# luo-ziyuan/NeRF_Signature

Hardware: AMD Instinct MI355X
Metric: training rays/sec @4096 rays (hotdog, 32-bit msg) (higher is better)
Workload: dtype f32 (hash gather, compositing) + fp16 MFMA with f32 accumulate (MLPs); 1 GPU; BASELINE configs[1]: Blender/hotdog-like S0, --wtmk_tcnn, 4096 content + 32x12x12 block rays, 32-bit msg; content_rays=4096, block_rays_total=4608, block_rays_this_rank=4608, message_dim=32, parallelism=dp1, capacity_overflow=False, recaptured_with_more_headroom_after_warmup=False, execution=hipgraph, graph_segments=1

## Files before the change

### include/nerfsig.h

```cpp
#ifndef NERFSIG_H_
#define NERFSIG_H_

#include <stddef.h>
#include <stdint.h>

#ifdef __cplusplus
extern "C" {
#endif

#define NSIG_OK 0
#define NSIG_ERR_ARG 1
#define NSIG_ERR_LAUNCH 2

#define NSIG_TABLE_ROWS (1u << 19)
#define NSIG_BASE_LEVELS 16
#define NSIG_MAX_MESSAGE_DIM 64

typedef void *nsig_stream_t;

int nsig_abi_version(void);
const char *nsig_last_error(void);


int rm_near_far_from_aabb(const float *rays_o, const float *rays_d, const float *aabb, uint32_t N, float min_near,
// ... 133 lines not shown
#define NSIG_PLANES_MIXED 1
int field_fwd(const float *xyzs, const float *dirs, uint32_t M, float bound, const float *const *base_tables_host,
              const float *S, const void *packed, float *sigmas, float *rgbs, float *geo_feat, uint32_t *masks,
              const void *planes, int planes_layout, nsig_stream_t stream);

size_t hg_planes_bytes(uint32_t M);
int hg_encode_planes(const float *xyzs, uint32_t M, float bound, const float *const *base_tables_host, const float *S,
                     void *planes, nsig_stream_t stream);
int hg_encode_planes_rows(const float *xyzs, uint32_t M_capacity, const uint32_t *rows_dev, float bound,
                          const float *const *base_tables_host, const float *S, void *planes, nsig_stream_t stream);
int hg_encode_planes_mixed(const float *xyzs, uint32_t M_capacity, const uint32_t *rows_dev, float bound, const float *const *base_tables_host,
                           const float *S, void *planes, nsig_stream_t stream);
int field_fwd_rows(const float *xyzs, const float *dirs, uint32_t M_capacity, const uint32_t *rows_dev, float bound,
                   const float *const *base_tables_host, const float *S, const void *packed, float *sigmas, float *rgbs, const void *planes,
                   int planes_layout, nsig_stream_t stream);

int hg_warm_tables(const float *const *base_tables_host, const float *S, float *sink, nsig_stream_t stream);

int hg_encode_codebook_plane(const float *xyzs, uint32_t M, float bound, const float *S, void *planes, int planes_layout, void *plan_to_reset,
                             nsig_stream_t stream);

int field_color_fwd(const float *dirs, const float *geo_feat, uint32_t M, const void *packed, float *rgbs,
                    nsig_stream_t stream);

int field_bwd(const float *xyzs, uint32_t M, float bound, const float *grad_sigmas, const float *grad_rgbs,
              const float *sigmas, const float *rgbs, const uint32_t *masks, const void *packed, float *G,
              float *dfeat_out, float *rec_out, nsig_stream_t stream);
int field_bwd_planned(const float *xyzs, uint32_t M, float bound, const float *grad_sigmas, const float *grad_rgbs,
                      const float *sigmas, const float *rgbs, const uint32_t *masks, const void *packed, void *plan,
                      nsig_stream_t stream);

int opt_adam_dense(uint32_t n, float *const *params_host, const float *const *grads_host, float *const *exp_avg_host,
                   float *const *exp_avg_sq_host, float *const *steps_host, const uint32_t *numel_host, const float *lr, float beta1,
                   float beta2, float eps, float grad_scale, float *scratch, nsig_stream_t stream);
int opt_adam_dense_host(uint32_t n, float *const *params_host, const float *const *grads_host, float *const *exp_avg_host,
// ... 122 lines not shown
```

### nerf_signature_amd/_native.py

```python
import ctypes
import os

import torch

_PKG = os.path.dirname(os.path.abspath(__file__))
LIB_PATH = os.path.join(_PKG, "lib", "libnerfsig.so")

_c = ctypes
_vp, _u32, _fl, _int, _sz = _c.c_void_p, _c.c_uint32, _c.c_float, _c.c_int, _c.c_size_t

SIGNATURES = {
    "nsig_abi_version": [],
    "nsig_last_error": [],
    "nsig_host_device_pointer": [_vp],
    "rg_sample_rays": [_vp, _u32, _vp, _fl, _fl, _fl, _fl, _u32, _u32, _u32, _vp, _u32, _u32, _c.c_uint64, _vp, _vp, _vp, _vp, _vp, _vp],
    "rg_get_rays": [_vp, _fl, _fl, _fl, _fl, _u32, _u32, _vp, _u32, _u32, _vp, _vp, _vp],
    "rm_near_far_from_aabb": [_vp, _vp, _vp, _u32, _fl, _vp, _vp, _vp],
    "rm_sph_from_ray": [_vp, _vp, _fl, _u32, _vp, _vp],
    "rm_morton3D": [_vp, _u32, _vp, _vp],
    "rm_morton3D_invert": [_vp, _u32, _vp, _vp],
    "rm_packbits": [_vp, _u32, _fl, _vp, _vp],
    "rg_refresh_draw_scratch_bytes": [_u32, _u32],
    "rg_refresh_begin": [_vp, _u32, _vp],
    "rg_refresh_draw": [_vp, _vp, _u32, _u32, _vp, _vp, _c.c_uint64, _vp, _u32, _vp],
# ... 9 lines not shown
    "rm_march_train_write": [_vp, _vp, _fl, _fl, _u32, _u32, _u32, _u32, _u32, _vp, _vp, _vp, _vp, _vp, _vp, _vp, _vp, _vp],
    "rm_march_train_count_nf": [_vp, _vp, _vp, _fl, _vp, _fl, _fl, _u32, _u32, _u32, _u32, _vp, _vp, _vp, _vp, _vp, _vp],
    "rm_march_train_scan_write_max_rays": [],
    "rm_march_train_scan_write": [_vp, _vp, _fl, _fl, _u32, _u32, _u32, _u32, _u32, _vp, _vp, _vp, _vp, _vp, _vp, _vp, _vp, _vp, _vp],
    "rm_composite_train_fwd": [_vp, _vp, _vp, _vp, _u32, _u32, _fl, _vp, _vp, _vp, _vp],
    "rm_composite_train_bwd": [_vp, _vp, _vp, _vp, _vp, _vp, _vp, _vp, _u32, _u32, _fl, _vp, _vp, _vp],
    "rm_march": [_u32, _u32, _vp, _vp, _vp, _vp, _fl, _fl, _u32, _u32, _u32, _vp, _vp, _vp, _vp, _vp, _vp, _vp, _u32, _vp],
    "rm_composite": [_u32, _u32, _fl, _vp, _vp, _vp, _vp, _vp, _vp, _vp, _vp, _vp],
    "rm_compact_alive": [_vp, _u32, _vp, _vp, _vp],
    "rm_eval_begin": [_u32, _vp, _vp, _vp],
    "rm_eval_march": [_vp, _u32, _vp, _vp, _vp, _vp, _fl, _fl, _u32, _u32, _u32, _vp, _vp, _vp, _vp, _vp, _vp, _vp],
    "rm_eval_composite": [_vp, _u32, _fl, _fl, _vp, _vp, _vp, _vp, _vp, _vp, _vp, _vp, _vp],
    "rm_eval_compact": [_vp, _u32, _u32, _vp, _vp, _vp],
    "hg_encode_planes_rows": [_vp, _u32, _vp, _fl, _vp, _vp, _vp, _vp],
    "hg_encode_planes_mixed": [_vp, _u32, _vp, _fl, _vp, _vp, _vp, _vp],
    "field_fwd_rows": [_vp, _vp, _u32, _vp, _fl, _vp, _vp, _vp, _vp, _vp, _vp, _int, _vp],
    "hg_codebook_presum": [_vp, _u32, _vp, _vp],
    "hg_codebook_presum_sel": [_vp, _vp, _u32, _vp, _vp],
    "hg_encode_fwd": [_vp, _u32, _vp, _vp, _vp, _vp],
    "hg_codebook_encode_fwd": [_vp, _u32, _vp, _u32, _vp, _vp],
    "hg_codebook_bwd": [_vp, _u32, _vp, _vp, _vp],
    "hg_scatter_sliced": [_vp, _u32, _vp, _vp],
    "hg_fanout_grad": [_vp, _vp, _u32, _int, _vp],
    "hg_level_lookup": [_vp, _u32, _fl, _vp, _vp, _vp],
    "opt_codebook_adam": [_vp, _vp, _vp, _vp, _u32, _fl, _fl, _fl, _vp, _vp, _fl, _vp],
    "opt_codebook_adam_sel": [_vp, _vp, _vp, _vp, _vp, _vp, _u32, _vp, _fl, _fl, _fl, _fl, _vp, _vp],
    "opt_codebook_adam_sel_next": [_vp, _vp, _vp, _vp, _vp, _vp, _u32, _vp, _fl, _fl, _fl, _fl, _vp, _vp, _vp, _vp],
    "mlp_packed_bytes": [],
    "mlp_get_precision": [],
    "mlp_set_precision": [_int],
    "mlp_get_pipelined": [],
    "mlp_set_pipelined": [_int],
    "mlp_pack_weights": [_vp, _vp, _vp, _vp],
    "hg_planes_bytes": [_u32],
    "hg_encode_planes": [_vp, _u32, _fl, _vp, _vp, _vp, _vp],
    "hg_warm_tables": [_vp, _vp, _vp, _vp],
    "hg_encode_codebook_plane": [_vp, _u32, _fl, _vp, _vp, _int, _vp, _vp],
    "field_fwd": [_vp, _vp, _u32, _fl, _vp, _vp, _vp, _vp, _vp, _vp, _vp, _vp, _int, _vp],
    "field_color_fwd": [_vp, _vp, _u32, _vp, _vp, _vp],
    "opt_adam_dense_host": [_u32, _vp, _vp, _vp, _vp, _vp, _vp, _vp, _fl, _fl, _fl, _fl, _vp],
    "opt_adam_dense": [_u32, _vp, _vp, _vp, _vp, _vp, _vp, _vp, _fl, _fl, _fl, _fl, _vp, _vp],
    "rm_composite_train_finish_fwd": [_vp, _vp, _vp, _vp, _u32, _u32, _fl, _vp, _vp, _vp, _u32, _vp, _vp, _vp, _vp, _vp, _vp],
    "rm_composite_train_finish_bwd": [_vp, _vp, _vp, _vp, _vp, _vp, _vp, _vp, _vp, _u32, _u32, _u32, _fl, _u32, _vp, _vp, _vp],
    "rm_finish_fwd": [_vp, _vp, _vp, _vp, _vp, _vp, _u32, _u32, _vp, _vp, _vp],
    "rm_finish_bwd": [_vp, _vp, _vp, _vp, _vp, _vp, _u32, _u32, _vp, _vp, _vp],
    "loop_step_begin": [_vp, _u32, _vp, _u32, _u32, _vp, _vp, _vp],
    "wm_loss_fwd": [_vp, _vp, _u32, _vp, _vp, _u32, _fl, _fl, _fl, _vp, _vp, _vp, _vp],
    "wm_loss_bwd": [_vp, _vp, _vp, _fl, _fl, _vp, _u32, _vp, _u32, _vp, _vp, _vp],
    "dec_bn_gelu_fwd": [_vp, _vp, _vp, _u32, _u32, _u32, _fl, _vp, _vp, _vp],
    "dec_bn_gelu_bwd": [_vp, _vp, _vp, _vp, _vp, _u32, _u32, _u32, _vp, _vp, _vp, _vp],
    "dec_workspace_bytes": [_u32, _u32, _u32, _u32],
    "dec_forward": [_vp, _u32, _vp, _vp, _vp, _u32, _u32, _u32, _u32, _fl, _vp, _vp, _vp, _vp],
# ... 134 lines not shown
```

### nerf_signature_amd/csrc/field.hip

```cpp
#include <cstdlib>
#include <cstring>
#include <mutex>
#include <unordered_set>
#include "fieldmlp.h"

#include <stdlib.h>

namespace nsig {


__device__ inline float fwd_weight(int frag, int lane, int j, const float *__restrict__ sp, const float *__restrict__ cp) {
    const int r = lane & 31, h = lane >> 5;
    if (frag < F1) {
        const int rb = (frag - F0) >> 1, ks = (frag - F0) & 1;
        return sp[kSigmaW1 + (32 * rb + r) * 32 + 16 * ks + 8 * h + j];
    }
    if (frag < F2) return r < 16 ? sp[kSigmaW2 + r * 64 + k_from_acc(frag - F1, h, j)] : 0.0f;
    if (frag < F3) {
        const int rb = (frag - F2) >> 1, ks = (frag - F2) & 1;
        int cin;
        if (ks == 0) cin = 8 * h + j;
        else { const int rho = row_of_reg(h, j); cin = rho == 0 ? 31 : 15 + rho; }
        return cp[kColorW1 + (32 * rb + r) * 32 + cin];
    }
// ... 136 lines not shown
        if (m >= lim) continue;
        const uint32_t ml = min(m, M - 1);
        const float3 pt = *reinterpret_cast<const float3 *>(xyzs + 3 * (size_t)ml);
        const float x = (pt.x + bound) / two_b, y = (pt.y + bound) / two_b, z = (pt.z + bound) / two_b;
        for (int i = 0; i < n_levels; ++i) {
            const int l = tab.level[slot][i];
            const bool half_out = mixed && l < kHalfLevels;
            float2 *out = !mixed ? planes + (size_t)l * stride + m
                                 : (half_out ? reinterpret_cast<float2 *>(reinterpret_cast<uint32_t *>(planes) + (size_t)l * stride + m) : mixed_f32_plane(planes, stride, l) + m);
            encode_tile_level(reinterpret_cast<const float2 *>(l == NSIG_BASE_LEVELS ? S : base.p[l]), geom.cell[l], xs, x, y, z, out, half_out, mixed);
        }
    }
}

__global__ void __launch_bounds__(256) k_encode_codebook_plane(const float *__restrict__ xyzs, uint32_t M, float bound, float cell, const float *__restrict__ S,
                                                               float2 *__restrict__ plane, uint32_t stride, BinHeader *__restrict__ reset) {
    if (reset != nullptr && blockIdx.x == 0 && threadIdx.x == 0) reset->gmax_bits = 0;
    const uint32_t m = blockIdx.x * 256 + threadIdx.x;
    if (m >= stride) return;
    const uint32_t ml = min(m, M - 1);
    const float two_b = 2.0f * bound;
    const float3 pt = *reinterpret_cast<const float3 *>(xyzs + 3 * (size_t)ml);
    const float x = (pt.x + bound) / two_b, y = (pt.y + bound) / two_b, z = (pt.z + bound) / two_b;
    encode_tile_level(reinterpret_cast<const float2 *>(S), cell, threadIdx.x & 1u, x, y, z, plane + m);
}

template <typename P, bool kMixed>
__device__ inline void field_fwd_pipelined(const char *lds, int lane, const float *__restrict__ dirs, uint32_t M, bool add_codebook,
                                           const float2 *__restrict__ planes, uint32_t stride, float *__restrict__ sigmas, float *__restrict__ rgbs,
                                           uint32_t *__restrict__ masks) {
    static_assert(!kMixed || P::kMfmaPerProduct == 1, "mixed plane sets carry fp16 operands: the fp16 MLP only");
    constexpr size_t kHalf = kFwdBytes;
    const int p = lane & 31, h = lane >> 5;
    const uint32_t n_tiles = ceil_div(M, 32u);
// ... 664 lines not shown
    NSIG_REQUIRE(sink != nullptr, "hg_warm_tables: sink is one writable float (never written)");
    TablePtrs base{};
    if (int e = fill_base_tables(base_tables_host, base, "hg_warm_tables")) return e;
    k_warm_tables<<<8 * 128, 256, 0, as_stream(stream)>>>(base, S, default_slots(S != nullptr), sink);
    return check_launch("hg_warm_tables");
}

NSIG_EXPORT size_t hg_planes_bytes(uint32_t M) { return (size_t)(NSIG_BASE_LEVELS + 1) * ceil_div(M, 32u) * 32u * sizeof(float2); }

static int check_layout(int layout, const char *who) {
    NSIG_REQUIRE(layout == NSIG_PLANES_F32 || layout == NSIG_PLANES_MIXED, "%s: planes_layout must be NSIG_PLANES_F32 (0) or NSIG_PLANES_MIXED (1)", who);
    return NSIG_OK;
}

static int encode_planes_impl(const float *xyzs, uint32_t M, float bound, const float *const *base_tables_host, const float *S, void *planes,
                              const uint32_t *rows_dev, nsig_stream_t stream, bool mixed = false) {
    if (M == 0) return NSIG_OK;
    NSIG_REQUIRE(xyzs && planes, "hg_encode_planes: null pointer");
    NSIG_REQUIRE(bound > 0.0f, "hg_encode_planes: bound must be positive");
    NSIG_REQUIRE((reinterpret_cast<uintptr_t>(planes) & 7) == 0, "hg_encode_planes: planes must be 8-byte aligned");
    TablePtrs base{};
    if (int e = fill_base_tables(base_tables_host, base, "hg_encode_planes")) return e;
    const uint32_t stride = ceil_div(M, 32u) * 32u;
    const SlotTable tab = default_slots(S != nullptr);
    int covered[NSIG_BASE_LEVELS + 1] = {};
    for (int s = 0; s < 8; ++s)
        for (int i = 0; i < tab.n[s]; ++i) covered[tab.level[s][i]] += 1;
    for (int l = 0; l < NSIG_BASE_LEVELS + (S != nullptr ? 1 : 0); ++l)
        NSIG_REQUIRE(covered[l] == 1, "hg_encode_planes: level %d is assigned to %d slots", l, covered[l]);
    NSIG_REQUIRE(S != nullptr || covered[NSIG_BASE_LEVELS] == 0, "hg_encode_planes: slot table names the codebook level but S is NULL");
    const uint32_t tiles = ceil_div(stride, 256u);
    const uint32_t per_slot = tiles < 8192u ? tiles : 8192u;
    if (mixed) k_encode_planes<true><<<per_slot * 8, 256, 0, as_stream(stream)>>>(xyzs, M, bound, base, make_level_geom(), S, reinterpret_cast<float2 *>(planes), stride, tab, rows_dev);
    else k_encode_planes<false><<<per_slot * 8, 256, 0, as_stream(stream)>>>(xyzs, M, bound, base, make_level_geom(), S, reinterpret_cast<float2 *>(planes), stride, tab, rows_dev);
    return check_launch("hg_encode_planes");
}

NSIG_EXPORT int hg_encode_planes_mixed(const float *xyzs, uint32_t M_capacity, const uint32_t *rows_dev, float bound, const float *const *base_tables_host,
                                       const float *S, void *planes, nsig_stream_t stream) {
    NSIG_REQUIRE(mlp_precision() == 1, "hg_encode_planes_mixed: the mixed layout carries the fp16 MLP's operands (mlp_set_precision(1))");
    return encode_planes_impl(xyzs, M_capacity, bound, base_tables_host, S, planes, rows_dev, stream, true);
}

NSIG_EXPORT int hg_encode_planes(const float *xyzs, uint32_t M, float bound, const float *const *base_tables_host, const float *S, void *planes,
                                 nsig_stream_t stream) {
    return encode_planes_impl(xyzs, M, bound, base_tables_host, S, planes, nullptr, stream);
}

NSIG_EXPORT int hg_encode_planes_rows(const float *xyzs, uint32_t M_capacity, const uint32_t *rows_dev, float bound, const float *const *base_tables_host,
                                      const float *S, void *planes, nsig_stream_t stream) {
    NSIG_REQUIRE(rows_dev != nullptr, "hg_encode_planes_rows: null row count");
    return encode_planes_impl(xyzs, M_capacity, bound, base_tables_host, S, planes, rows_dev, stream);
}

NSIG_EXPORT int hg_encode_codebook_plane(const float *xyzs, uint32_t M, float bound, const float *S, void *planes, int planes_layout, void *plan_to_reset,
                                         nsig_stream_t stream) {
    if (M == 0) return NSIG_OK;
    if (int e = check_layout(planes_layout, "hg_encode_codebook_plane")) return e;
    NSIG_REQUIRE(xyzs && S && planes, "hg_encode_codebook_plane: null pointer");
    NSIG_REQUIRE(bound > 0.0f, "hg_encode_codebook_plane: bound must be positive");
    NSIG_REQUIRE((reinterpret_cast<uintptr_t>(planes) & 7) == 0, "hg_encode_codebook_plane: planes must be 8-byte aligned");
    NSIG_REQUIRE(plan_to_reset == nullptr || (reinterpret_cast<uintptr_t>(plan_to_reset) & 15) == 0, "hg_encode_codebook_plane: plan must be 16-byte aligned");
    const uint32_t stride = ceil_div(M, 32u) * 32u;
    float2 *plane = planes_layout == NSIG_PLANES_MIXED ? mixed_f32_plane(planes, stride, NSIG_BASE_LEVELS) : reinterpret_cast<float2 *>(planes) + (size_t)NSIG_BASE_LEVELS * stride;
    k_encode_codebook_plane<<<ceil_div(stride, 256u), 256, 0, as_stream(stream)>>>(xyzs, M, bound, make_level_geom().cell[NSIG_BASE_LEVELS], S, plane, stride,
                                                                                  reinterpret_cast<BinHeader *>(plan_to_reset));
    return check_launch("hg_encode_codebook_plane");
}

static int field_fwd_impl(const float *xyzs, const float *dirs, uint32_t M, float bound, const float *const *base_tables_host,
                          const float *S, const void *packed, float *sigmas, float *rgbs, float *geo_feat, uint32_t *masks,
                          const void *planes, int planes_layout, const uint32_t *rows_dev, nsig_stream_t stream) {
    if (M == 0) return NSIG_OK;
    NSIG_REQUIRE(xyzs && packed && sigmas, "field_fwd: null pointer");
    NSIG_REQUIRE(rgbs == nullptr || dirs != nullptr, "field_fwd: dirs is required when rgbs is requested");
    NSIG_REQUIRE(bound > 0.0f, "field_fwd: bound must be positive");
    NSIG_REQUIRE((reinterpret_cast<uintptr_t>(packed) & 15) == 0, "field_fwd: packed must be 16-byte aligned");
    TablePtrs base{};
    if (int e = fill_base_tables(base_tables_host, base, "field_fwd")) return e;
    const char *pk = reinterpret_cast<const char *>(packed);
    hipStream_t st = as_stream(stream);
    const bool f16 = mlp_precision() == 1;
// ... 151 lines not shown
```

### nerf_signature_amd/fieldops.py

```python
import os

import torch
from torch.autograd import Function
from torch.amp import custom_bwd, custom_fwd

from . import _native as nv

T_ROWS = 1 << 19
MASK_WORDS = 6

_fwd32 = custom_fwd(device_type="cuda", cast_inputs=torch.float32)
_bwd = custom_bwd(device_type="cuda")


def message_bits(message):
    if message is None:
        return None
    if isinstance(message, torch.Tensor):
        return tuple(int(v) for v in message.detach().to("cpu", torch.float32).tolist())
    return tuple(int(v) for v in message)


def select_tables(tables, bits):
    if len(tables) != 2 * len(bits):
# ... 96 lines not shown
def field_forward(xyzs, dirs, bound, base_tables, S, packed, want_rgb=True, want_geo=False, want_masks=False, planes=None, fixed=None):
    xyzs = xyzs.contiguous().float()
    M, dev = xyzs.shape[0], xyzs.device
    sigmas = torch.empty(M, dtype=torch.float32, device=dev)
    rgbs = torch.empty(M, 3, dtype=torch.float32, device=dev) if want_rgb else None
    geo = torch.empty(M, 15, dtype=torch.float32, device=dev) if want_geo else None
    masks = torch.empty((M + 31) // 32 * 32, MASK_WORDS, dtype=torch.int32, device=dev) if want_masks else None
    if want_rgb:
        dirs = dirs.contiguous().float()
    use_planes = (M >= PLANES_MIN_POINTS) if planes is None else bool(planes)
    base_ptrs = nv.ptr_array([_check_table(t.detach(), "base table") for t in base_tables])
    ws, layout = None, PLANES_F32
    if fixed is not None:
        fixed.check(xyzs, bound, base_tables)
        ws, layout = fixed.planes, fixed.layout
        reset = nv.ptr(fixed.plan.buf) if want_masks else None
        if S is not None:
            nv.call("hg_encode_codebook_plane", nv.ptr(xyzs), M, float(bound), nv.ptr(S), nv.ptr(ws), layout, reset, nv.stream())
    elif use_planes:
        ws = torch.empty(int(nv.fn("hg_planes_bytes")(M)), dtype=torch.uint8, device=dev)
        layout = encode_planes(xyzs, M, bound, base_ptrs, S, ws)
    nv.call("field_fwd", nv.ptr(xyzs), nv.ptr(dirs) if want_rgb else None, M, float(bound), base_ptrs, nv.ptr(S), nv.ptr(packed),
            nv.ptr(sigmas), nv.ptr(rgbs), nv.ptr(geo), nv.ptr(masks), nv.ptr(ws), layout, nv.stream())
    return sigmas, rgbs, geo, masks


def field_color(dirs, geo_feat, packed):
    dirs = dirs.contiguous().float()
    geo_feat = geo_feat.contiguous().float()
    M = dirs.shape[0]
    rgbs = torch.empty(M, 3, dtype=torch.float32, device=dirs.device)
# ... 104 lines not shown
                torch.cuda.current_stream().wait_event(self.ready)
            self.ready = None


class _KeptPlan:

    def __init__(self, M, buf):
        self.M, self.buf, self.launched, self.ready = M, buf, True, None

    def join(self):
        pass


class FixedPoints:

    def __init__(self, xyzs, bound, base_tables):
        self.M, self.bound = int(xyzs.shape[0]), float(bound)
        self.xyzs_ptr = xyzs.data_ptr()
        self.planes = torch.empty(int(nv.fn("hg_planes_bytes")(self.M)), dtype=torch.uint8, device=xyzs.device)
        self.plan = _KeptPlan(self.M, torch.empty(int(nv.fn("hg_scatter_plan_bytes")(self.M)), dtype=torch.uint8, device=xyzs.device))
        self.refreshes = 0
        self.refresh(xyzs, base_tables)

    @staticmethod
    def _tables_key(base_tables):
        return tuple((t.data_ptr(), t._version) for t in base_tables) + (mixed_planes(),)

    def refresh(self, xyzs, base_tables):
        if xyzs.data_ptr() != self.xyzs_ptr or xyzs.shape[0] != self.M:
            raise ValueError("FixedPoints.refresh: these are not the points the cache was built for")
        base_ptrs = nv.ptr_array([_check_table(t.detach(), "base table") for t in base_tables])
        self.layout = encode_planes(xyzs, self.M, self.bound, base_ptrs, None, self.planes)
        nv.call("hg_scatter_plan", nv.ptr(xyzs), self.M, self.bound, nv.ptr(self.plan.buf), nv.stream())
        self.key = self._tables_key(base_tables)
        self.refreshes += 1

    def check(self, xyzs, bound, base_tables):
        if xyzs.data_ptr() != self.xyzs_ptr or xyzs.shape[0] != self.M or float(bound) != self.bound:
            raise ValueError("FixedPoints: the field pass was handed other points than the cache was built for")
        if self._tables_key(base_tables) != self.key and not torch.cuda.is_current_stream_capturing():
            self.refresh(xyzs, base_tables)


def field_backward_planned(xyzs, bound, g_sigma, g_rgb, sigmas, rgbs, masks, packed, plan, G):
    plan.join()
    nv.call("field_bwd_planned", nv.ptr(xyzs), plan.M, float(bound), nv.ptr(g_sigma.contiguous().float()), nv.ptr(g_rgb.contiguous().float()),
            nv.ptr(sigmas), nv.ptr(rgbs), nv.ptr(masks), nv.ptr(packed), nv.ptr(plan.buf), nv.stream())
    nv.call("hg_scatter_planned", nv.ptr(plan.buf), plan.M, nv.ptr(G), nv.stream())
# ... 74 lines not shown
    __slots__ = ("base", "sel")

    def __init__(self, base, sel):
        self.base, self.sel = list(base), list(sel)


class _FieldFunction(Function):

    @staticmethod
    @_fwd32
    def forward(ctx, xyzs, dirs, bound, packed, S, sink, tabs, fixed, *diff):
        base, sel = tabs.base, tabs.sel
        n_sel = len(sel)
        need_grad = n_sel > 0 and len(diff) > 0
        xyzs = xyzs.contiguous().float()
        if fixed is not None:
            ctx.plan = fixed.plan if need_grad else None
        else:
            ctx.plan = ScatterPlan(xyzs, bound) if need_grad and xyzs.shape[0] >= binned_min_points() else None
        sigmas, rgbs, _, masks = field_forward(xyzs, dirs, bound, base, S, packed, want_masks=need_grad, fixed=fixed)
        ctx.bound, ctx.n_diff, ctx.need_grad, ctx.sink = bound, len(diff), need_grad, sink
        if need_grad:
            ctx.mlp_precision = nv.fn("mlp_get_precision")()
            ctx.save_for_backward(xyzs, sigmas, rgbs, masks, packed)
            if sink is not None:
                sink.selected = list(sel)
                ctx.sink_selected = sink.selected
        return sigmas, rgbs

    @staticmethod
    @_bwd
# ... 137 lines not shown
```

### nerf_signature_amd/network.py

```python
import torch

from . import fieldops as fo
from . import tcnn_compat as tcnn
from .hash_encoding import HashEmbedder
from .hash_encoding_wtmk_bit import HashEmbedder as HashEmbedder_msg
from .hidden_models import get_hidden_decoder_multi_views, normalize_img
from .renderer import NeRFRenderer


def _data_parallel():
    import torch.distributed as dist
    return dist.is_available() and dist.is_initialized() and dist.get_world_size() > 1


class NeRFNetwork(NeRFRenderer):
    def __init__(self, num_layers=2, hidden_dim=64, geo_feat_dim=15, num_layers_color=3, hidden_dim_color=64, bound=1, message_dim=16,
                 n_views=1, finetune_decoder=False, **kwargs):
        super().__init__(bound, **kwargs)
        if (num_layers, hidden_dim, geo_feat_dim, num_layers_color, hidden_dim_color) != (2, 64, 15, 3, 64):
            raise NotImplementedError("the native field network implements the reference's default architecture: "
                                      "sigma 32->64->1+15, color 16+15->64->64->3")
        self.finetune_decoder = finetune_decoder
        self.num_layers, self.hidden_dim, self.geo_feat_dim = num_layers, hidden_dim, geo_feat_dim
        self.num_layers_color, self.hidden_dim_color = num_layers_color, hidden_dim_color
# ... 178 lines not shown
        if capacity is None:
            capacity = self._count_points(o, d, dt_gamma, max_steps)
        rec = self.march_ahead(rays_o, rays_d, dt_gamma, max_steps, capacity=capacity)
        if loop_capacity is None and int(rec["counter"][0]) > capacity:
            capacity = raymarching.padded_point_count(int(rec["counter"][0]))
            rec = self.march_ahead(rays_o, rays_d, dt_gamma, max_steps, capacity=capacity)
        if rec.get("fixed") is None:
            rec["fixed"] = fo.FixedPoints(rec["xyzs"], self.bound, self.encoder.tables())
        else:
            rec["fixed"].refresh(rec["xyzs"], self.encoder.tables())
        rec["fixed_args"] = (dt_gamma, max_steps)
        rec["rays_ref"] = (rays_o, rays_d)
        rec["grid_key"] = self.grid_key()
        return rec

    def density(self, x, message=None):
        selected, _, S = self._select(message)
        if torch.is_grad_enabled() and x.is_cuda and len(selected) and any(t.requires_grad for t in selected):
            sigma, geo = fo.density_apply(x, self.bound, self._packed(), self.encoder.tables(), selected, S, self.grad_sink, self.sigma_net.params)
            return {"sigma": sigma, "geo_feat": geo}
        sigma, _, geo, _ = fo.field_forward(x, None, self.bound, self.encoder.tables(), S, self._packed(), want_rgb=False, want_geo=True)
        return {"sigma": sigma, "geo_feat": geo}

    def color(self, x, d, mask=None, geo_feat=None, **kwargs):
        grad = torch.is_grad_enabled() and geo_feat is not None and geo_feat.requires_grad and d.is_cuda
        one = (lambda dd, gg: fo.color_apply(dd, gg, self._packed(), self.color_net.params)) if grad else (lambda dd, gg: fo.field_color(dd, gg, self._packed()))
        if mask is not None:
            rgbs = torch.zeros(mask.shape[0], 3, dtype=torch.float32, device=x.device)
            if not mask.any():
                return rgbs
# ... 13 lines not shown
```

### nerf_signature_amd/renderer.py

```python
import math
import os

import numpy as np
import torch
import torch.nn as nn

from . import _native as nv
from . import raymarching


def custom_meshgrid(*args):
    return torch.meshgrid(*args, indexing="ij")


def sample_pdf(bins, weights, n_samples, det=False):
    B, T = bins.shape
    mass = weights + 1e-5
    cdf = torch.zeros(B, T, dtype=mass.dtype, device=mass.device)
    torch.cumsum(mass / mass.sum(-1, keepdim=True), -1, out=cdf[:, 1:])
    if det:
        q = ((torch.arange(n_samples, dtype=mass.dtype) + 0.5) / n_samples).to(mass.device).expand(B, n_samples)
    else:
        q = torch.rand(B, n_samples).to(mass.device)
    q = q.contiguous()
# ... 229 lines not shown
        if differentiable:
            rgbs = rgb_all * (weights > 1e-4).unsqueeze(-1)
        else:
            rgbs = self.color(pts.reshape(-1, 3), dirs_of(pts), mask=(weights > 1e-4).reshape(-1), geo_feat=geo.reshape(N * T, -1)).view(N, T, 3)
        weights_sum = weights.sum(dim=-1)
        depth = torch.sum(weights * ((z - nears) / span).clamp(0, 1), dim=-1)
        image = torch.sum(weights.unsqueeze(-1) * rgbs, dim=-2) + (1 - weights_sum).unsqueeze(-1) * bg_color
        return {"depth": depth.view(*prefix), "image": image.view(*prefix, 3), "weights_sum": weights_sum}



    @staticmethod
    def _rays_key(o, d):
        return (o.data_ptr(), o._version, d.data_ptr(), d._version, o.shape[0])

    def march_ahead(self, rays_o, rays_d, dt_gamma=0, max_steps=1024, perturb=False, phase="all", capacity=None, noises=None):
        if not hasattr(self, "_marched"):
            self._marched = {}
        prefix, o, d = self._flatten_rays(rays_o, rays_d)
        if capacity is None:
            capacity = getattr(self, "point_capacity", None)
            capacity = capacity.get(o.shape[0]) if capacity else None
        if capacity is None or not o.is_cuda:
            raise RuntimeError("march_ahead needs point_capacity for this ray count (see trainer.GraphedWatermarkLoop.prepare) and CUDA rays")
        rec = next((r for r in self._marched.values() if r["ptrs"] == (o.data_ptr(), d.data_ptr(), o.shape[0]) and r["capacity"] == capacity), None)
        if rec is None:
            N, dev = o.shape[0], o.device
            f32 = dict(dtype=torch.float32, device=dev)
            rec = {"ptrs": (o.data_ptr(), d.data_ptr(), N), "capacity": capacity, "nears": torch.empty(N, **f32), "fars": torch.empty(N, **f32),
                   "xyzs": torch.empty(capacity, 3, **f32), "dirs": torch.empty(capacity, 3, **f32), "deltas": torch.empty(capacity, 2, **f32),
                   "rays": torch.empty(N, 3, dtype=torch.int32, device=dev), "counter": torch.zeros(2, dtype=torch.int32, device=dev), "key": None,
                   "counts": torch.empty(N, dtype=torch.int32, device=dev), "t_rec": torch.empty(N * int(max_steps), **f32), "max_steps": int(max_steps),
                   "noises": None}
        if rec["max_steps"] != int(max_steps):
            raise ValueError("march_ahead: max_steps changed for rays that were marched before")
        N = o.shape[0]
        geom = (float(self.bound), float(dt_gamma), int(max_steps), N, int(self.cascade), int(self.grid_size))
        if phase in ("all", "count") and not raymarching.fused_limits():
            raymarching.near_far_into(o, d, self.aabb_train, self.min_near, rec["nears"], rec["fars"])
            rec["noises"] = noises if noises is not None else (torch.rand(N, dtype=torch.float32, device=o.device) if perturb else None)
            nv.call("rm_march_train_count", nv.ptr(o), nv.ptr(d), nv.ptr(self.density_bitfield), *geom, nv.ptr(rec["nears"]), nv.ptr(rec["fars"]),
                    nv.ptr(rec["noises"]), nv.ptr(rec["counts"]), nv.ptr(rec["t_rec"]), nv.stream())
        elif phase in ("all", "count"):
            rec["noises"] = noises if noises is not None else (torch.rand(N, dtype=torch.float32, device=o.device) if perturb else None)
            nv.call("rm_march_train_count_nf", nv.ptr(o), nv.ptr(d), nv.ptr(self.aabb_train), float(self.min_near), nv.ptr(self.density_bitfield), *geom,
                    nv.ptr(rec["noises"]), nv.ptr(rec["nears"]), nv.ptr(rec["fars"]), nv.ptr(rec["counts"]), nv.ptr(rec["t_rec"]), nv.stream())
        if phase in ("all", "write"):
            if N <= raymarching.scan_write_max_rays():
                nv.call("rm_march_train_scan_write", nv.ptr(o), nv.ptr(d), geom[0], geom[1], geom[2], N, geom[4], geom[5], capacity, nv.ptr(rec["nears"]),
                        nv.ptr(rec["noises"]), nv.ptr(rec["t_rec"]), nv.ptr(rec["counts"]), nv.ptr(rec["rays"]), nv.ptr(rec["counter"]), nv.ptr(rec["xyzs"]),
                        nv.ptr(rec["dirs"]), nv.ptr(rec["deltas"]), nv.stream())
            else:
                nv.call("rm_march_train_scan", nv.ptr(rec["counts"]), N, nv.ptr(rec["rays"]), nv.ptr(rec["counter"]), nv.stream())
                nv.call("rm_march_train_write", nv.ptr(o), nv.ptr(d), geom[0], geom[1], geom[2], N, geom[4], geom[5], capacity, nv.ptr(rec["nears"]),
                        nv.ptr(rec["noises"]), nv.ptr(rec["t_rec"]), nv.ptr(rec["rays"]), nv.ptr(rec["counter"]), nv.ptr(rec["xyzs"]), nv.ptr(rec["dirs"]),
                        nv.ptr(rec["deltas"]), nv.stream())
        self._marched = {k: r for k, r in self._marched.items() if r is not rec}
        rec["key"] = self._rays_key(o, d)
        self._marched[rec["key"]] = rec
        return rec

    def drop_marched(self):
        self._marched = {}

    def premarch(self, rays_o, rays_d, dt_gamma=0, max_steps=1024):
        import weakref
        prefix, o, d = self._flatten_rays(rays_o, rays_d)
        nears, fars = raymarching.near_far_from_aabb(o, d, self.aabb_train, self.min_near)
        counter = self.step_counter[self.local_step % 16]
        self.local_step += 1
        counter.zero_()
# ... 40 lines not shown
            if bg is not None:
                weights_sum, depth, image = out
                return {"depth": depth.view(*prefix), "image": image.view(*prefix, 3), "weights_sum": weights_sum}
            weights_sum, depth, image = out
        else:
            weights_sum, depth, image = self._march_and_composite_eval(o, d, message, nears, fars, dt_gamma, perturb, max_steps, T_thresh)
        image, depth = self._finish(prefix, image, depth, weights_sum, bg_color, nears, fars)
        results = {"depth": depth, "image": image}
        if self.training:
            results["weights_sum"] = weights_sum
        return results

    def _march_and_composite_train(self, o, d, message, nears, fars, dt_gamma, perturb, force_all_rays, max_steps, T_thresh, finish=None,
                                   marched=None, limits=None):
        if marched is not None:
            fixed = marched.get("fixed")
            if fixed is not None:
                sigmas, rgbs = self(marched["xyzs"], marched["dirs"], message, fixed=fixed)
            else:
                sigmas, rgbs = self(marched["xyzs"], marched["dirs"], message)
            sigmas = sigmas if self.density_scale == 1 else self.density_scale * sigmas
            if finish is not None:
                return _CompositeFinish.apply(sigmas, rgbs, marched["deltas"], marched["rays"], nears, fars, finish, T_thresh)
            return raymarching.composite_rays_train(sigmas, rgbs, marched["deltas"], marched["rays"], T_thresh)
        counter = self.step_counter[self.local_step % 16]
        self.local_step += 1
        capacity = getattr(self, "point_capacity", None)
        capacity = capacity.get(o.shape[0]) if capacity else None
        if not (capacity is not None and force_all_rays):
            counter.zero_()
        if capacity is not None and force_all_rays:
            xyzs, dirs, deltas, rays = raymarching.march_rays_train_capacity(o, d, self.bound, self.density_bitfield, self.cascade,
                                                                            self.grid_size, nears, fars, counter, capacity, perturb,
# ... 253 lines not shown
```

### nerf_signature_amd/trainer.py

```python
import ctypes
import os

import numpy as np
import torch
import torch.nn.functional as F

from . import _native as nv
from . import fieldops as fo
from . import dp
from .capture import SegmentedCapture, warm_up
from .dp import GradExchange, exchange_active, world_size
from .distortion import DistortionLayer, host_uniform, scaled_width
from .hidden_models import normalize_img, set_grad_arena, set_weights_stream


def loss_w_bce(decoded, keys, temp=10.0):
    return F.binary_cross_entropy_with_logits(decoded * temp, keys, reduction="mean")


def loss_w_mse(decoded, keys, temp=10.0):
    return torch.mean((decoded * temp - (2 * keys - 1)) ** 2)


class _WatermarkLoss(torch.autograd.Function):
# ... 336 lines not shown
        p = preds.detach().cpu().numpy() if torch.is_tensor(preds) else preds
        t = truths.detach().cpu().numpy() if torch.is_tensor(truths) else truths
        self.V += -10 * np.log10(np.mean((p - t) ** 2))
        self.N += 1

    def measure(self):
        return self.V / self.N

    def report(self):
        return f"PSNR = {self.measure():.6f}"


class GraphedWatermarkLoop:

    def __init__(self, model, optimizer, render_kwargs, data, lambda_w=1.0, lambda_i=1.0, lr_lambda=None, headroom=0.0, overlap_content=True,
                 content_headroom=None, content_sampler=None, fixed_blocks=False, distortion="none", distortion_seed=0):
        self.distortion = None if distortion in (None, "none") else (distortion if isinstance(distortion, DistortionLayer) else DistortionLayer(distortion, distortion_seed))
        self.fixed_blocks = bool(fixed_blocks)
        self._refix_pending = False
        self._kept_key = None
        self.content_sampler = content_sampler
        self._s_for = None
        self.marched = None
        self._pending_content = None
        self.side_stream = torch.cuda.Stream() if overlap_content else None
        self.plan_stream = self.side_stream
        self.weights_stream = self.side_stream
        self.content_backward_first = False
        if not hasattr(optimizer, "step_shared_sel"):
            raise TypeError("GraphedWatermarkLoop needs nerf_signature_amd.optim.CodebookAdam(capturable=True)")
        if not any(t.requires_grad for t in model.msg_encoder.tables()):
            raise NotImplementedError("GraphedWatermarkLoop captures the step that trains the codebook; with a frozen codebook "
                                      "(finetune_decoder=True) drive the model with WatermarkLoop")
        self.model, self.optimizer = model, optimizer
        self.render_kwargs = dict(render_kwargs)
        self.lambda_w, self.lambda_i = lambda_w, lambda_i
        self.lr_lambda, self.headroom = lr_lambda, headroom
        self.content_headroom = headroom if content_headroom is None else content_headroom
# ... 32 lines not shown
            model._graphed_loops = []
        model._graphed_loops.append(self)

    def resume_at(self, step):
        if self.selected is not None and self._replays:
            raise RuntimeError("resume_at: the loop has already replayed steps")
        self.steps_done = int(step)
        self._replays = int(step)
        self.stage_counter.fill_(int(step))

    def invalidate(self):
        self._s_for = None
        self.model._packed()
        if self.fixed_blocks and self.selected is not None:
            self._fix_blocks()

    @torch.no_grad()
    def gather_codebook(self, optimizer_state=True):
        if self.opt_shard is None:
            return
        import torch.distributed as dist
        from .optim import _prepare_device_state
        b0, b1 = self.opt_shard
        world = dist.get_world_size()
        _prepare_device_state(self.optimizer, self.tables)
        kinds = [lambda t: t.data]
        if optimizer_state:
            dp_state = self.optimizer.state
            kinds += [lambda t, k=k: dp_state[t][k] for k in ("exp_avg", "exp_avg_sq", "step") if all(k in dp_state[t] for t in self.tables)]
        for get in kinds:
# ... 64 lines not shown
        import torch.distributed as dist
        post = lambda: dp.collective(lambda: dist.all_reduce(S, op=dist.ReduceOp.SUM), last=True, name="all_reduce_presum")
        if defer_collective:
            return post
        post()
        return None

    def _march_ahead(self):
        kw, wm = self.render_kwargs, self.data["watermark"]
        args = (kw.get("dt_gamma", 0), kw.get("max_steps", 1024))
        block_o, block_d, _ = local_blocks(wm)
        if self.fixed_blocks:
            self.marched = self.marched[:1]
        else:
            self.marched = (self.model.march_ahead(block_o, block_d, *args),)

    @torch.no_grad()
    def _fix_blocks(self):
        kw = self.render_kwargs
        block_o, block_d, _ = local_blocks(self.data["watermark"])
        rec = self.model.fix_rays(block_o, block_d, kw.get("dt_gamma", 0), kw.get("max_steps", 1024))
        self.marched = (rec,) + tuple(self.marched[1:] if self.marched else ())
        self._refix_pending = False
        self._kept_key = self._kept_inputs_key()

    def _optimise_and_march(self):
        if not self.march_ahead or self.fixed_blocks:
            return self._optimise()
        main = torch.cuda.current_stream()
        self.side_stream.wait_stream(main)
        with torch.cuda.stream(self.side_stream):
            self._march_ahead()
            self._warm_tables()
        post = self._optimise(defer_collective=True)
        main.wait_stream(self.side_stream)
        if post is not None:
            post()

    def _warm_tables(self):
        if self.opt_shard is not None or self.fixed_blocks or getattr(self.model, "_presum_cache", None) is None:
            return
        tables = nv.ptr_array([t.detach() for t in self.model.encoder.tables()])
        nv.call("hg_warm_tables", tables, nv.ptr(self.model._presum_cache[1]), nv.ptr(self._warm_sink), nv.stream())

    def point_counts(self):
        if self.marched is not None:
            return int(self.marched[0]["counter"][0]), int(self.model.step_counter[self.capacity_rows[-1], 0])
        a, b = self.model.step_counter[self.capacity_rows, 0].tolist()
        return (a, b) if self._blocks_issued_first() else (b, a)

    def _blocks_issued_first(self):
        return self.side_stream is None or self.content_backward_first

    def _kept_inputs_key(self):
        m = self.model
        return m.grid_key() + tuple((t.data_ptr(), t._version) for t in m.encoder.tables())

    def _set_inputs(self, message, data, next_data=None, next_message=None, eager_copy=True):
        if self.fixed_blocks and self.selected is not None and not self._refix_pending and self._kept_key != self._kept_inputs_key():
            self._refix_pending = True
        if self._refix_pending:
            self._fix_blocks()
        slot = self._replays % len(self.msg_ring)
        if self.msg_events[slot] is not None:
            self.msg_events[slot].synchronize()
        D = self.msg_dev.numel()
        self.msg_ring[slot][:D].copy_(message.detach().to("cpu", torch.float32))
        self.msg_ring[slot][D:2 * D].copy_((message if next_message is None else next_message).detach().to("cpu", torch.float32))
        if self.lr_lambda is not None:
            self.msg_ring[slot][2 * D] = self.base_lr * self.lr_lambda(self.steps_done)
        if eager_copy:
            self.msg_all[:self.stage_width].copy_(self.msg_ring[slot][:self.stage_width], non_blocking=True)
            ev = torch.cuda.Event()
            ev.record()
            self.msg_events[slot] = ev
        if self._pending_content is not None:
            for k, v in self._pending_content.items():
# ... 78 lines not shown
        self.capacity_rows, self.capacities = v["capacity_rows"], v["capacities"]

    @property
    def segments(self):
        return self.selected.segments if self.selected is not None else []

    @property
    def between(self):
        return self.selected.between if self.selected is not None else []

    @property
    def graphs(self):
        return tuple(self.selected.segments) if self.selected is not None else None

    @property
    def march_ahead(self):
        return self.side_stream is not None

    def _warm_up_step(self):
        self.optimizer.zero_grad(set_to_none=True)
        self._forward_backward()
        self.exchange(self.sink.G)
        self._optimise()

    def _captured_step(self):
        out = self._forward_backward()
        self.exchange(self.sink.G)
        self._optimise_and_march()
        return out

    def _segment_ended(self):
        fo.forget_plan_events()
# ... 3 lines not shown
        slot = self._replays % len(self.msg_ring)
        self._replays += 1
        if self.stage_in_graph:
            ev = torch.cuda.Event()
            ev.record()
            self.msg_events[slot] = ev

    def _capture(self, cap_block, cap_content):
        model = self.model
        self.optimizer.zero_grad(set_to_none=True)
        if self.march_ahead and not self.fixed_blocks:
            self._march_ahead()
        if self._capture_stream is None:
            self._capture_stream = torch.cuda.Stream()
        capture = SegmentedCapture(self._capture_stream, on_boundary=self._segment_ended, after_first=self._first_segment_replayed)
        out = capture.capture(self._captured_step)
        capacity_rows = [(model.local_step - 2) % 16, (model.local_step - 1) % 16]
        self.content_capacity = cap_content
        if self.marched is not None:
            capacity_rows = [(model.local_step - 1) % 16]
        return {"capture": capture, "out": out, "capacity_rows": capacity_rows,
                "capacities": [cap_block, cap_content] if self._blocks_issued_first() else [cap_content, cap_block]}

    def step(self, message, data=None, next_data=None, next_message=None):
        if self.selected is None:
            if data is not None:
                self._set_inputs(message, data)
                data = None
            self.prepare(message)
        unannounced = self._s_for is None or not torch.equal(self._s_for, message.detach().to("cpu", torch.float32))
        self._set_inputs(message, data, next_data, next_message, eager_copy=unannounced or not self.stage_in_graph)
# ... 42 lines not shown
```

Measured before the change: 4.462 million rays/s.

## Pre-gather next step's base hash planes on a side stream mid-step

Adds an 'ahead' path that, right after the field forward of the block rays, marches the next step's block rays into staging buffers on a separate stream. It also pre-encodes their base-level hash planes using a capped number of workgroups, so this work overlaps with the decoder and backward on the main stream. The staged march results are promoted at optimiser time instead of re-marching. The per-step codebook plane is then the only level encoded on the critical path, and table warming is skipped. Risks: stale base tables, since the planes are gathered before the optimiser updates them, extra staging copies, and contention with main-stream kernels.

```diff
diff --git a/include/nerfsig.h b/include/nerfsig.h
--- a/include/nerfsig.h
+++ b/include/nerfsig.h
@@ -171,11 +171,15 @@
 int field_fwd_rows(const float *xyzs, const float *dirs, uint32_t M_capacity, const uint32_t *rows_dev, float bound,
                    const float *const *base_tables_host, const float *S, const void *packed, float *sigmas, float *rgbs, const void *planes,
                    int planes_layout, nsig_stream_t stream);
+int hg_encode_base_planes_beside(const float *xyzs, uint32_t M, float bound, const float *const *base_tables_host, void *planes, int planes_layout,
+                                 uint32_t wgs_per_slot, nsig_stream_t stream);
 
 int hg_warm_tables(const float *const *base_tables_host, const float *S, float *sink, nsig_stream_t stream);
 
 int hg_encode_codebook_plane(const float *xyzs, uint32_t M, float bound, const float *S, void *planes, int planes_layout, void *plan_to_reset,
                              nsig_stream_t stream);
+int hg_encode_codebook_plane_rows(const float *xyzs, uint32_t M_capacity, const uint32_t *rows_dev, float bound, const float *S, void *planes,
+                                  int planes_layout, void *plan_to_reset, nsig_stream_t stream);
 
 int field_color_fwd(const float *dirs, const float *geo_feat, uint32_t M, const void *packed, float *rgbs,
                     nsig_stream_t stream);
diff --git a/nerf_signature_amd/_native.py b/nerf_signature_amd/_native.py
--- a/nerf_signature_amd/_native.py
+++ b/nerf_signature_amd/_native.py
@@ -47,6 +47,7 @@
     "rm_eval_compact": [_vp, _u32, _u32, _vp, _vp, _vp],
     "hg_encode_planes_rows": [_vp, _u32, _vp, _fl, _vp, _vp, _vp, _vp],
     "hg_encode_planes_mixed": [_vp, _u32, _vp, _fl, _vp, _vp, _vp, _vp],
+    "hg_encode_base_planes_beside": [_vp, _u32, _fl, _vp, _vp, _int, _u32, _vp],
     "field_fwd_rows": [_vp, _vp, _u32, _vp, _fl, _vp, _vp, _vp, _vp, _vp, _vp, _int, _vp],
     "hg_codebook_presum": [_vp, _u32, _vp, _vp],
     "hg_codebook_presum_sel": [_vp, _vp, _u32, _vp, _vp],
@@ -69,6 +70,7 @@
     "hg_encode_planes": [_vp, _u32, _fl, _vp, _vp, _vp, _vp],
     "hg_warm_tables": [_vp, _vp, _vp, _vp],
     "hg_encode_codebook_plane": [_vp, _u32, _fl, _vp, _vp, _int, _vp, _vp],
+    "hg_encode_codebook_plane_rows": [_vp, _u32, _vp, _fl, _vp, _vp, _int, _vp, _vp],
     "field_fwd": [_vp, _vp, _u32, _fl, _vp, _vp, _vp, _vp, _vp, _vp, _vp, _vp, _int, _vp],
     "field_color_fwd": [_vp, _vp, _u32, _vp, _vp, _vp],
     "opt_adam_dense_host": [_u32, _vp, _vp, _vp, _vp, _vp, _vp, _vp, _fl, _fl, _fl, _fl, _vp],
diff --git a/nerf_signature_amd/csrc/field.hip b/nerf_signature_amd/csrc/field.hip
--- a/nerf_signature_amd/csrc/field.hip
+++ b/nerf_signature_amd/csrc/field.hip
@@ -174,10 +174,18 @@
 }
 
 __global__ void __launch_bounds__(256) k_encode_codebook_plane(const float *__restrict__ xyzs, uint32_t M, float bound, float cell, const float *__restrict__ S,
-                                                               float2 *__restrict__ plane, uint32_t stride, BinHeader *__restrict__ reset) {
+                                                               float2 *__restrict__ plane, uint32_t stride, BinHeader *__restrict__ reset,
+                                                               const uint32_t *__restrict__ rows_dev) {
     if (reset != nullptr && blockIdx.x == 0 && threadIdx.x == 0) reset->gmax_bits = 0;
+    uint32_t lim = stride;
+    if (rows_dev != nullptr) {
+        const uint32_t r = *rows_dev;
+        if (r == 0) return;
+        M = min(M, r);
+        lim = min(stride, ceil_div(M, 32u) * 32u);
+    }
     const uint32_t m = blockIdx.x * 256 + threadIdx.x;
-    if (m >= stride) return;
+    if (m >= lim) return;
     const uint32_t ml = min(m, M - 1);
     const float two_b = 2.0f * bound;
     const float3 pt = *reinterpret_cast<const float3 *>(xyzs + 3 * (size_t)ml);
@@ -872,7 +880,7 @@
 }
 
 static int encode_planes_impl(const float *xyzs, uint32_t M, float bound, const float *const *base_tables_host, const float *S, void *planes,
-                              const uint32_t *rows_dev, nsig_stream_t stream, bool mixed = false) {
+                              const uint32_t *rows_dev, nsig_stream_t stream, bool mixed = false, uint32_t wgs_per_slot = 0) {
     if (M == 0) return NSIG_OK;
     NSIG_REQUIRE(xyzs && planes, "hg_encode_planes: null pointer");
     NSIG_REQUIRE(bound > 0.0f, "hg_encode_planes: bound must be positive");
@@ -888,7 +896,8 @@
         NSIG_REQUIRE(covered[l] == 1, "hg_encode_planes: level %d is assigned to %d slots", l, covered[l]);
     NSIG_REQUIRE(S != nullptr || covered[NSIG_BASE_LEVELS] == 0, "hg_encode_planes: slot table names the codebook level but S is NULL");
     const uint32_t tiles = ceil_div(stride, 256u);
-    const uint32_t per_slot = tiles < 8192u ? tiles : 8192u;
+    uint32_t per_slot = tiles < 8192u ? tiles : 8192u;
+    if (wgs_per_slot != 0 && wgs_per_slot < per_slot) per_slot = wgs_per_slot;
     if (mixed) k_encode_planes<true><<<per_slot * 8, 256, 0, as_stream(stream)>>>(xyzs, M, bound, base, make_level_geom(), S, reinterpret_cast<float2 *>(planes), stride, tab, rows_dev);
     else k_encode_planes<false><<<per_slot * 8, 256, 0, as_stream(stream)>>>(xyzs, M, bound, base, make_level_geom(), S, reinterpret_cast<float2 *>(planes), stride, tab, rows_dev);
     return check_launch("hg_encode_planes");
@@ -900,6 +909,13 @@
     return encode_planes_impl(xyzs, M_capacity, bound, base_tables_host, S, planes, rows_dev, stream, true);
 }
 
+NSIG_EXPORT int hg_encode_base_planes_beside(const float *xyzs, uint32_t M, float bound, const float *const *base_tables_host, void *planes, int planes_layout,
+                                             uint32_t wgs_per_slot, nsig_stream_t stream) {
+    if (int e = check_layout(planes_layout, "hg_encode_base_planes_beside")) return e;
+    NSIG_REQUIRE(planes_layout != NSIG_PLANES_MIXED || mlp_precision() == 1, "hg_encode_base_planes_beside: the mixed layout carries the fp16 MLP's operands (mlp_set_precision(1))");
+    return encode_planes_impl(xyzs, M, bound, base_tables_host, nullptr, planes, nullptr, stream, planes_layout == NSIG_PLANES_MIXED, wgs_per_slot);
+}
+
 NSIG_EXPORT int hg_encode_planes(const float *xyzs, uint32_t M, float bound, const float *const *base_tables_host, const float *S, void *planes,
                                  nsig_stream_t stream) {
     return encode_planes_impl(xyzs, M, bound, base_tables_host, S, planes, nullptr, stream);
@@ -911,8 +927,8 @@
     return encode_planes_impl(xyzs, M_capacity, bound, base_tables_host, S, planes, rows_dev, stream);
 }
 
-NSIG_EXPORT int hg_encode_codebook_plane(const float *xyzs, uint32_t M, float bound, const float *S, void *planes, int planes_layout, void *plan_to_reset,
-                                         nsig_stream_t stream) {
+static int encode_codebook_plane_impl(const float *xyzs, uint32_t M, const uint32_t *rows_dev, float bound, const float *S, void *planes, int planes_layout,
+                                      void *plan_to_reset, nsig_stream_t stream) {
     if (M == 0) return NSIG_OK;
     if (int e = check_layout(planes_layout, "hg_encode_codebook_plane")) return e;
     NSIG_REQUIRE(xyzs && S && planes, "hg_encode_codebook_plane: null pointer");
@@ -922,8 +938,19 @@
     const uint32_t stride = ceil_div(M, 32u) * 32u;
     float2 *plane = planes_layout == NSIG_PLANES_MIXED ? mixed_f32_plane(planes, stride, NSIG_BASE_LEVELS) : reinterpret_cast<float2 *>(planes) + (size_t)NSIG_BASE_LEVELS * stride;
     k_encode_codebook_plane<<<ceil_div(stride, 256u), 256, 0, as_stream(stream)>>>(xyzs, M, bound, make_level_geom().cell[NSIG_BASE_LEVELS], S, plane, stride,
-                                                                                  reinterpret_cast<BinHeader *>(plan_to_reset));
+                                                                                  reinterpret_cast<BinHeader *>(plan_to_reset), rows_dev);
     return check_launch("hg_encode_codebook_plane");
+}
+
+NSIG_EXPORT int hg_encode_codebook_plane(const float *xyzs, uint32_t M, float bound, const float *S, void *planes, int planes_layout, void *plan_to_reset,
+                                         nsig_stream_t stream) {
+    return encode_codebook_plane_impl(xyzs, M, nullptr, bound, S, planes, planes_layout, plan_to_reset, stream);
+}
+
+NSIG_EXPORT int hg_encode_codebook_plane_rows(const float *xyzs, uint32_t M_capacity, const uint32_t *rows_dev, float bound, const float *S, void *planes,
+                                              int planes_layout, void *plan_to_reset, nsig_stream_t stream) {
+    NSIG_REQUIRE(rows_dev != nullptr, "hg_encode_codebook_plane_rows: null row count");
+    return encode_codebook_plane_impl(xyzs, M_capacity, rows_dev, bound, S, planes, planes_layout, plan_to_reset, stream);
 }
 
 static int field_fwd_impl(const float *xyzs, const float *dirs, uint32_t M, float bound, const float *const *base_tables_host,
diff --git a/nerf_signature_amd/fieldops.py b/nerf_signature_amd/fieldops.py
--- a/nerf_signature_amd/fieldops.py
+++ b/nerf_signature_amd/fieldops.py
@@ -134,7 +134,7 @@
     if fixed is not None:
         fixed.check(xyzs, bound, base_tables)
         ws, layout = fixed.planes, fixed.layout
-        reset = nv.ptr(fixed.plan.buf) if want_masks else None
+        reset = nv.ptr(fixed.plan.buf) if want_masks and fixed.plan is not None else None
         if S is not None:
             nv.call("hg_encode_codebook_plane", nv.ptr(xyzs), M, float(bound), nv.ptr(S), nv.ptr(ws), layout, reset, nv.stream())
     elif use_planes:
@@ -269,11 +269,11 @@
 
 class FixedPoints:
 
-    def __init__(self, xyzs, bound, base_tables):
+    def __init__(self, xyzs, bound, base_tables, keep_plan=True):
         self.M, self.bound = int(xyzs.shape[0]), float(bound)
         self.xyzs_ptr = xyzs.data_ptr()
         self.planes = torch.empty(int(nv.fn("hg_planes_bytes")(self.M)), dtype=torch.uint8, device=xyzs.device)
-        self.plan = _KeptPlan(self.M, torch.empty(int(nv.fn("hg_scatter_plan_bytes")(self.M)), dtype=torch.uint8, device=xyzs.device))
+        self.plan = _KeptPlan(self.M, torch.empty(int(nv.fn("hg_scatter_plan_bytes")(self.M)), dtype=torch.uint8, device=xyzs.device)) if keep_plan else None
         self.refreshes = 0
         self.refresh(xyzs, base_tables)
 
@@ -281,12 +281,17 @@
     def _tables_key(base_tables):
         return tuple((t.data_ptr(), t._version) for t in base_tables) + (mixed_planes(),)
 
-    def refresh(self, xyzs, base_tables):
-        if xyzs.data_ptr() != self.xyzs_ptr or xyzs.shape[0] != self.M:
+    def refresh(self, xyzs, base_tables, staged=False, wgs_per_slot=0):
+        if (xyzs.data_ptr() != self.xyzs_ptr and not staged) or xyzs.shape[0] != self.M:
             raise ValueError("FixedPoints.refresh: these are not the points the cache was built for")
         base_ptrs = nv.ptr_array([_check_table(t.detach(), "base table") for t in base_tables])
-        self.layout = encode_planes(xyzs, self.M, self.bound, base_ptrs, None, self.planes)
-        nv.call("hg_scatter_plan", nv.ptr(xyzs), self.M, self.bound, nv.ptr(self.plan.buf), nv.stream())
+        if wgs_per_slot:
+            self.layout = PLANES_MIXED if mixed_planes() else PLANES_F32
+            nv.call("hg_encode_base_planes_beside", nv.ptr(xyzs), self.M, self.bound, base_ptrs, nv.ptr(self.planes), self.layout, int(wgs_per_slot), nv.stream())
+        else:
+            self.layout = encode_planes(xyzs, self.M, self.bound, base_ptrs, None, self.planes)
+        if self.plan is not None:
+            nv.call("hg_scatter_plan", nv.ptr(xyzs), self.M, self.bound, nv.ptr(self.plan.buf), nv.stream())
         self.key = self._tables_key(base_tables)
         self.refreshes += 1
 
@@ -391,7 +396,7 @@
         n_sel = len(sel)
         need_grad = n_sel > 0 and len(diff) > 0
         xyzs = xyzs.contiguous().float()
-        if fixed is not None:
+        if fixed is not None and fixed.plan is not None:
             ctx.plan = fixed.plan if need_grad else None
         else:
             ctx.plan = ScatterPlan(xyzs, bound) if need_grad and xyzs.shape[0] >= binned_min_points() else None
diff --git a/nerf_signature_amd/network.py b/nerf_signature_amd/network.py
--- a/nerf_signature_amd/network.py
+++ b/nerf_signature_amd/network.py
@@ -216,6 +216,13 @@
         rec["grid_key"] = self.grid_key()
         return rec
 
+    def gather_ahead(self, rec):
+        if rec.get("ahead") is None:
+            rec["ahead"] = fo.FixedPoints(rec["xyzs"], self.bound, self.encoder.tables(), keep_plan=False)
+        else:
+            rec["ahead"].refresh(rec["xyzs"], self.encoder.tables())
+        return rec["ahead"]
+
     def density(self, x, message=None):
         selected, _, S = self._select(message)
         if torch.is_grad_enabled() and x.is_cuda and len(selected) and any(t.requires_grad for t in selected):
diff --git a/nerf_signature_amd/renderer.py b/nerf_signature_amd/renderer.py
--- a/nerf_signature_amd/renderer.py
+++ b/nerf_signature_amd/renderer.py
@@ -267,7 +267,20 @@
     def _rays_key(o, d):
         return (o.data_ptr(), o._version, d.data_ptr(), d._version, o.shape[0])
 
-    def march_ahead(self, rays_o, rays_d, dt_gamma=0, max_steps=1024, perturb=False, phase="all", capacity=None, noises=None):
+    STAGED_KEYS = ("nears", "fars", "xyzs", "dirs", "deltas", "rays", "counter")
+
+    @staticmethod
+    def staging_buffers(rec):
+        if rec.get("staged") is None:
+            rec["staged"] = {k: torch.empty_like(rec[k]) for k in ("nears", "fars", "xyzs", "dirs", "deltas", "rays", "counts", "t_rec")}
+            rec["staged"].update(counter=torch.zeros_like(rec["counter"]), noises=None)
+        return rec["staged"]
+
+    def promote_staged(self, rec):
+        for k in self.STAGED_KEYS:
+            rec[k].copy_(rec["staged"][k])
+
+    def march_ahead(self, rays_o, rays_d, dt_gamma=0, max_steps=1024, perturb=False, phase="all", capacity=None, noises=None, staged=False):
         if not hasattr(self, "_marched"):
             self._marched = {}
         prefix, o, d = self._flatten_rays(rays_o, rays_d)
@@ -287,6 +300,9 @@
                    "noises": None}
         if rec["max_steps"] != int(max_steps):
             raise ValueError("march_ahead: max_steps changed for rays that were marched before")
+        owner = rec
+        if staged:
+            rec = self.staging_buffers(owner)
         N = o.shape[0]
         geom = (float(self.bound), float(dt_gamma), int(max_steps), N, int(self.cascade), int(self.grid_size))
         if phase in ("all", "count") and not raymarching.fused_limits():
@@ -308,6 +324,8 @@
                 nv.call("rm_march_train_write", nv.ptr(o), nv.ptr(d), geom[0], geom[1], geom[2], N, geom[4], geom[5], capacity, nv.ptr(rec["nears"]),
                         nv.ptr(rec["noises"]), nv.ptr(rec["t_rec"]), nv.ptr(rec["rays"]), nv.ptr(rec["counter"]), nv.ptr(rec["xyzs"]), nv.ptr(rec["dirs"]),
                         nv.ptr(rec["deltas"]), nv.stream())
+        if staged:
+            return rec
         self._marched = {k: r for k, r in self._marched.items() if r is not rec}
         rec["key"] = self._rays_key(o, d)
         self._marched[rec["key"]] = rec
@@ -378,9 +396,11 @@
     def _march_and_composite_train(self, o, d, message, nears, fars, dt_gamma, perturb, force_all_rays, max_steps, T_thresh, finish=None,
                                    marched=None, limits=None):
         if marched is not None:
-            fixed = marched.get("fixed")
+            fixed = marched.get("fixed") or marched.get("ahead")
             if fixed is not None:
                 sigmas, rgbs = self(marched["xyzs"], marched["dirs"], message, fixed=fixed)
+                if marched.get("after_field") is not None:
+                    marched["after_field"]()
             else:
                 sigmas, rgbs = self(marched["xyzs"], marched["dirs"], message)
             sigmas = sigmas if self.density_scale == 1 else self.density_scale * sigmas
diff --git a/nerf_signature_amd/trainer.py b/nerf_signature_amd/trainer.py
--- a/nerf_signature_amd/trainer.py
+++ b/nerf_signature_amd/trainer.py
@@ -374,14 +374,21 @@
 class GraphedWatermarkLoop:
 
     def __init__(self, model, optimizer, render_kwargs, data, lambda_w=1.0, lambda_i=1.0, lr_lambda=None, headroom=0.0, overlap_content=True,
-                 content_headroom=None, content_sampler=None, fixed_blocks=False, distortion="none", distortion_seed=0):
+                 content_headroom=None, content_sampler=None, fixed_blocks=False, distortion="none", distortion_seed=0, base_ahead=True, ahead_placement="decoder"):
         self.distortion = None if distortion in (None, "none") else (distortion if isinstance(distortion, DistortionLayer) else DistortionLayer(distortion, distortion_seed))
         self.fixed_blocks = bool(fixed_blocks)
+        self._base_ahead = bool(base_ahead)
+        if ahead_placement not in ("decoder", "optimiser"):
+            raise ValueError("ahead_placement: 'decoder' | 'optimiser'")
+        self.ahead_placement = ahead_placement
+        self.ahead_wgs_per_slot = 128
+        self.ahead_stream = torch.cuda.Stream() if (overlap_content and base_ahead and ahead_placement == "decoder") else None
         self._refix_pending = False
         self._kept_key = None
         self.content_sampler = content_sampler
         self._s_for = None
         self.marched = None
+        self._ahead_mid_step_issued = False
         self._pending_content = None
         self.side_stream = torch.cuda.Stream() if overlap_content else None
         self.plan_stream = self.side_stream
@@ -444,6 +451,8 @@
         self.model._packed()
         if self.fixed_blocks and self.selected is not None:
             self._fix_blocks()
+        if self.base_ahead and self.selected is not None and self.marched is not None:
+            self.model.gather_ahead(self.marched[0])
 
     @torch.no_grad()
     def gather_codebook(self, optimizer_state=True):
@@ -538,6 +547,10 @@
             self.marched = self.marched[:1]
         else:
             self.marched = (self.model.march_ahead(block_o, block_d, *args),)
+            if self.base_ahead:
+                self.model.gather_ahead(self.marched[0])
+            else:
+                self.marched[0].pop("ahead", None)
 
     @torch.no_grad()
     def _fix_blocks(self):
@@ -548,13 +561,26 @@
         self._refix_pending = False
         self._kept_key = self._kept_inputs_key()
 
+    def _ahead_mid_step(self):
+        kw, rec = self.render_kwargs, self.marched[0]
+        block_o, block_d, _ = local_blocks(self.data["watermark"])
+        self.ahead_stream.wait_stream(torch.cuda.current_stream())
+        with torch.cuda.stream(self.ahead_stream):
+            staged = self.model.march_ahead(block_o, block_d, kw.get("dt_gamma", 0), kw.get("max_steps", 1024), staged=True)
+            rec["ahead"].refresh(staged["xyzs"], self.model.encoder.tables(), staged=True, wgs_per_slot=self.ahead_wgs_per_slot)
+
     def _optimise_and_march(self):
         if not self.march_ahead or self.fixed_blocks:
             return self._optimise()
         main = torch.cuda.current_stream()
         self.side_stream.wait_stream(main)
         with torch.cuda.stream(self.side_stream):
-            self._march_ahead()
+            if self._ahead_mid_step_issued:
+                self.side_stream.wait_stream(self.ahead_stream)
+                self.model.promote_staged(self.marched[0])
+                self._ahead_mid_step_issued = False
+            else:
+                self._march_ahead()
             self._warm_tables()
         post = self._optimise(defer_collective=True)
         main.wait_stream(self.side_stream)
@@ -562,7 +588,7 @@
             post()
 
     def _warm_tables(self):
-        if self.opt_shard is not None or self.fixed_blocks or getattr(self.model, "_presum_cache", None) is None:
+        if self.opt_shard is not None or self.fixed_blocks or self.base_ahead or getattr(self.model, "_presum_cache", None) is None:
             return
         tables = nv.ptr_array([t.detach() for t in self.model.encoder.tables()])
         nv.call("hg_warm_tables", tables, nv.ptr(self.model._presum_cache[1]), nv.ptr(self._warm_sink), nv.stream())
@@ -585,6 +611,9 @@
             self._refix_pending = True
         if self._refix_pending:
             self._fix_blocks()
+        ahead = self.marched[0].get("ahead") if self.base_ahead and self.selected is not None and self.marched else None
+        if ahead is not None and ahead.key != ahead._tables_key(self.model.encoder.tables()):
+            self.model.gather_ahead(self.marched[0])
         slot = self._replays % len(self.msg_ring)
         if self.msg_events[slot] is not None:
             self.msg_events[slot].synchronize()
@@ -693,8 +722,16 @@
         return tuple(self.selected.segments) if self.selected is not None else None
 
     @property
+    def base_ahead(self):
+        return self._base_ahead and self.march_ahead and not self.fixed_blocks and self.opt_shard is None and not self.sharded and world_size() == 1
+
+    @property
     def march_ahead(self):
         return self.side_stream is not None
+
+    def _note_mid_step(self):
+        self._ahead_mid_step()
+        self._ahead_mid_step_issued = True
 
     def _warm_up_step(self):
         self.optimizer.zero_grad(set_to_none=True)
@@ -728,7 +765,15 @@
         if self._capture_stream is None:
             self._capture_stream = torch.cuda.Stream()
         capture = SegmentedCapture(self._capture_stream, on_boundary=self._segment_ended, after_first=self._first_segment_replayed)
-        out = capture.capture(self._captured_step)
+        mid_step = self.base_ahead and self.ahead_stream is not None
+        if mid_step:
+            self.model.staging_buffers(self.marched[0])
+            self.marched[0]["after_field"] = self._note_mid_step
+        try:
+            out = capture.capture(self._captured_step)
+        finally:
+            if mid_step:
+                self.marched[0].pop("after_field", None)
         capacity_rows = [(model.local_step - 2) % 16, (model.local_step - 1) % 16]
         self.content_capacity = cap_content
         if self.marched is not None:
```

Result: slower. 3.509 million rays/s (-21.3%).
